# architector1324/micro-raytracer

Measured on AMD Instinct MI355X. Metric: Msamples/sec (res x spp), higher is better.
Workload: dtype f32

## Files before the change

micro_raytracer_amd/csrc/mrt_math.h:

```cpp
#pragma once

#include <stdint.h>

#if defined(__HIPCC__) || defined(__HIP__)
#define MRT_HD __host__ __device__ inline __attribute__((always_inline))
#define MRT_HD_NOINLINE __host__ __device__
#else
#define MRT_HD inline __attribute__((always_inline))
#define MRT_HD_NOINLINE
#endif

namespace mrt {

typedef uint32_t u32;
typedef int32_t i32;

MRT_HD u32 f2u(float f) { return __builtin_bit_cast(u32, f); }
MRT_HD float u2f(u32 u) { return __builtin_bit_cast(float, u); }
MRT_HD float fabs_(float x) { return __builtin_fabsf(x); }
MRT_HD float floor_(float x) { return __builtin_floorf(x); }
MRT_HD float trunc_(float x) { return __builtin_truncf(x); }

#if defined(__HIP_DEVICE_COMPILE__) && !defined(MRT_GENERIC_IEEE)
#define MRT_FAST_IEEE 1
MRT_HD bool wave_all(bool ok) { return __builtin_amdgcn_ballot_w64(!ok) == 0ull; }
#else
MRT_HD bool wave_all(bool ok) { return ok; }
#endif
constexpr float kWinLo = 0x1p-40f, kWinHi = 0x1p+40f;
MRT_HD bool in_window(float x) { const float a = fabs_(x); return a >= kWinLo && a <= kWinHi; }
MRT_HD bool in_window_pos(float x) { return x >= kWinLo && x <= kWinHi; }

#if defined(MRT_FAST_IEEE)
MRT_HD float sqrt_core_(float x)
{
    const float s = __builtin_amdgcn_sqrtf(x);
    const float sd = u2f(f2u(s) - 1u), su = u2f(f2u(s) + 1u);
    const float vd = __builtin_fmaf(-sd, s, x), vu = __builtin_fmaf(-su, s, x);
    float r = (0.0f >= vd) ? sd : s;
    r = (0.0f < vu) ? su : r;
    return r;
}
MRT_HD float rcp_refined_(float d)
{
    const float r0 = __builtin_amdgcn_rcpf(d);
    const float e = __builtin_fmaf(-d, r0, 1.0f);
    return __builtin_fmaf(e, r0, r0);
}
MRT_HD float div_core_(float n, float d, float r)
{
    const float q0 = n * r;
    const float q1 = __builtin_fmaf(__builtin_fmaf(-d, q0, n), r, q0);
    return __builtin_fmaf(__builtin_fmaf(-d, q1, n), r, q1);
}
#endif

MRT_HD float sqrt_(float x)
{
#if defined(MRT_FAST_IEEE)
    if (wave_all(in_window_pos(x))) return sqrt_core_(x);
#endif
    return __builtin_sqrtf(x);
}
MRT_HD float recip_(float x)
{
#if defined(MRT_FAST_IEEE)
    if (wave_all(in_window(x))) return div_core_(1.0f, x, rcp_refined_(x));
#endif
    return 1.0f / x;
}
MRT_HD float div_(float a, float b)
{
#if defined(MRT_FAST_IEEE)
    if (wave_all(in_window(a) && in_window(b))) return div_core_(a, b, rcp_refined_(b));
#endif
    return a / b;
}
MRT_HD void div2_(float a0, float a1, float b, float &q0, float &q1)
{
#if defined(MRT_FAST_IEEE)
    if (wave_all(in_window(a0) && in_window(a1) && in_window(b))) {
        const float r = rcp_refined_(b);
        q0 = div_core_(a0, b, r);
        q1 = div_core_(a1, b, r);
        return;
    }
#endif
    q0 = a0 / b;
    q1 = a1 / b;
}
MRT_HD float recip_sqrt_(float m)
{
#if defined(MRT_FAST_IEEE)
    if (wave_all(in_window_pos(m))) {
        const float s = sqrt_core_(m);
        return div_core_(1.0f, s, rcp_refined_(s));
    }
#endif
    return 1.0f / __builtin_sqrtf(m);
}
MRT_HD float rcp_fast(float x)
{
#if defined(__HIP_DEVICE_COMPILE__)
    return __builtin_amdgcn_rcpf(x);
#else
    return 1.0f / x;
#endif
}
MRT_HD float fma_(float a, float b, float c) { return __builtin_fmaf(a, b, c); }
MRT_HD float fma_fast(float a, float b, float c)
{
#if defined(__HIP_DEVICE_COMPILE__)
    return __builtin_fmaf(a, b, c);
#else
    return a * b + c;
#endif
}

constexpr float kPi = 3.14159274101257324f;
constexpr float kPiO2 = 1.57079637050628662f;
constexpr float kPiO4 = 0.785398185253143311f;
constexpr float kInf = __builtin_huge_valf();

MRT_HD float qnan() { return u2f(0x7fc00000u); }

#if defined(__HIP_DEVICE_COMPILE__)
MRT_HD float fmax_(float a, float b) { return __builtin_fmaxf(a, b); }
MRT_HD float fmin_(float a, float b) { return __builtin_fminf(a, b); }
#else
MRT_HD float fmax_(float a, float b)
{
    if (a != a) return b;
    if (b != b) return a;
    if (a == b) return (f2u(a) & 0x80000000u) ? b : a;
    return a < b ? b : a;
}
MRT_HD float fmin_(float a, float b)
{
    if (a != a) return b;
    if (b != b) return a;
    if (a == b) return (f2u(a) & 0x80000000u) ? a : b;
    return b < a ? b : a;
}
#endif

MRT_HD void sincos_(float x, float &s, float &c)
{
    if (!(fabs_(x) <= 65536.0f)) { s = qnan(); c = qnan(); return; }
    const float kf = floor_(fma_(x, 0.636619746685028076f, 0.5f));
    float r = fma_(-kf, 1.5703125f, x);
    r = fma_(-kf, 4.83751296997070312e-4f, r);
    r = fma_(-kf, 7.54978995489188216e-8f, r);
    const float z = r * r;
    const float sp = fma_(fma_(fma_(-1.9515295891e-4f, z, 8.3321608736e-3f), z, -1.6666654611e-1f) * z, r, r);
    const float cp = fma_(fma_(fma_(2.443315711809948e-5f, z, -1.388731625493765e-3f), z, 4.166664568298827e-2f) * z, z,
                          fma_(-0.5f, z, 1.0f));
    const int q = (int)kf & 3;
    float ss = (q & 1) ? cp : sp;
    float cc = (q & 1) ? sp : cp;
    if (q & 2) ss = -ss;
    if ((q + 1) & 2) cc = -cc;
    s = ss;
    c = cc;
}

MRT_HD float asin_core_(float a)
{
    const float z = a * a;
    const float p = fma_(fma_(fma_(fma_(4.2163199048e-2f, z, 2.4181311049e-2f), z, 4.5470025998e-2f), z, 7.4953002686e-2f), z, 1.6666752422e-1f);
    return fma_(p * z, a, a);
}

MRT_HD float acos_(float x)
{
    const float ax = fabs_(x);
    const bool big = ax > 0.5f;
    const float s = sqrt_(0.5f * (1.0f - ax));
    const float p = asin_core_(big ? s : x);
    const float two_p = 2.0f * p;
    const float r_big = (x > 0.0f) ? two_p : kPi - two_p;
    return big ? r_big : kPiO2 - p;
}

MRT_HD float atan_pos_(float t)
{
    float y0, x;
    if (t > 2.414213562373095f) { y0 = kPiO2; x = -recip_(t); }
    else if (t > 0.4142135623730950f) { y0 = kPiO4; x = div_(t - 1.0f, t + 1.0f); }
    else { y0 = 0.0f; x = t; }
    const float z = x * x;
    const float p = fma_(fma_(fma_(8.05374449538e-2f, z, -1.38776856032e-1f), z, 1.99777106478e-1f), z, -3.33329491539e-1f);
    return y0 + fma_(p * z, x, x);
}

MRT_HD float atan2_(float y, float x)
{
    if (x != x || y != y) return qnan();
    const float ay = fabs_(y), ax = fabs_(x);
    float a;
    if (ax == 0.0f) {
        if (ay == 0.0f) return 0.0f;
        a = kPiO2;
    } else if (ay == kInf && ax == kInf) {
        a = kPiO4;
    } else {
        a = atan_pos_(div_(ay, ax));
    }
    if (x < 0.0f) a = kPi - a;
    return (y < 0.0f) ? -a : a;
}

MRT_HD float pow_(float xf, float yf)
{
    if (yf == 0.0f) return 1.0f;
    if (xf != xf || yf != yf) return qnan();
    if (xf < 0.0f) return qnan();
    if (xf == 0.0f) return (yf > 0.0f) ? 0.0f : kInf;
    if (xf == kInf) return (yf > 0.0f) ? kInf : 0.0f;
    if (xf == 1.0f) return 1.0f;
    if (yf == kInf) return (xf > 1.0f) ? kInf : 0.0f;
    if (yf == -kInf) return (xf > 1.0f) ? 0.0f : kInf;

    const double x = (double)xf;
    const uint64_t bits = __builtin_bit_cast(uint64_t, x);
    int e = (int)((bits >> 52) & 0x7ff) - 1023;
    double m = __builtin_bit_cast(double, (bits & 0x000fffffffffffffULL) | 0x3ff0000000000000ULL);
    if (m > 1.4142135623730951) { m = m * 0.5; e = e + 1; }
    const double r = (m - 1.0) / (m + 1.0);
    const double r2 = r * r;
    double p = 1.0 / 23.0;
    p = p * r2 + 1.0 / 21.0;
    p = p * r2 + 1.0 / 19.0;
    p = p * r2 + 1.0 / 17.0;
    p = p * r2 + 1.0 / 15.0;
    p = p * r2 + 1.0 / 13.0;
    p = p * r2 + 1.0 / 11.0;
    p = p * r2 + 1.0 / 9.0;
    p = p * r2 + 1.0 / 7.0;
    p = p * r2 + 1.0 / 5.0;
    p = p * r2 + 1.0 / 3.0;
    p = p * r2 + 1.0;
    const double lnm = 2.0 * r * p;
    const double log2x = (double)e + lnm * 1.4426950408889634;
    const double t = (double)yf * log2x;
    if (t >= 129.0) return kInf;
    if (t <= -151.0) return 0.0f;
    const double kf = __builtin_floor(t + 0.5);
    const double f = (t - kf) * 0.6931471805599453;
    double q = 1.0 / 6227020800.0;
    q = q * f + 1.0 / 479001600.0;
    q = q * f + 1.0 / 39916800.0;
    q = q * f + 1.0 / 3628800.0;
    q = q * f + 1.0 / 362880.0;
    q = q * f + 1.0 / 40320.0;
    q = q * f + 1.0 / 5040.0;
    q = q * f + 1.0 / 720.0;
    q = q * f + 1.0 / 120.0;
    q = q * f + 1.0 / 24.0;
    q = q * f + 1.0 / 6.0;
    q = q * f + 0.5;
    q = q * f + 1.0;
    q = q * f + 1.0;
    const int k = (int)kf;
    const double scale = __builtin_bit_cast(double, (uint64_t)(k + 1023) << 52);
    return (float)(q * scale);
}

MRT_HD u32 mix32(u32 x)
{
    x ^= x >> 16; x *= 0x7feb352du; x ^= x >> 15; x *= 0x846ca68bu; x ^= x >> 16;
    return x;
}
constexpr u32 kGold = 0x9E3779B9u;
MRT_HD u32 path_key(u32 seed_lo, u32 seed_hi, u32 pixel, u32 sample)
{
    return mix32((mix32(pixel + seed_lo) ^ seed_hi) + sample * kGold);
}
MRT_HD u32 draw_u32(u32 pk, u32 dim) { return mix32(pk + (dim + 1u) * kGold); }
MRT_HD float u32_to_unit(u32 u) { return (float)(u >> 9) * 1.1920928955078125e-7f; }

enum : u32 { DIM_LENS_X = 0, DIM_LENS_Z = 1, DIM_BOUNCE0 = 2, DIMS_PER_BOUNCE = 8 };
enum : u32 { SL_REFL_COIN = 0, SL_REFL_U1, SL_REFL_U2, SL_OPAC_COIN, SL_REFR_COIN, SL_REFR_U1, SL_REFR_U2, SL_EMIT_COIN };

MRT_HD bool bernoulli(float p, u32 u)
{
    if (p == 1.0f) return true;
    return u < (u32)(p * 4294967296.0f);
}

MRT_HD i32 total_key(float t)
{
    if (t != t) return (i32)0x80000000u;
    i32 i = (i32)f2u(t);
    i ^= (i32)(((u32)(i >> 31)) >> 1);
    return i;
}

}
```

micro_raytracer_amd/csrc/mrt_trace.h:

```cpp
#pragma once
#include "mrt_scene.h"

namespace mrt {

#ifndef MRT_LEAF_QUEUE
#define MRT_LEAF_QUEUE 8u
#endif
constexpr u32 kLeafQueue = MRT_LEAF_QUEUE;

#ifndef MRT_PROBE
#define MRT_PROBE(phase)
#endif
#ifndef MRT_COUNT
#define MRT_COUNT(counter)
#endif
#ifndef MRT_PROBE_INST
#define MRT_PROBE_INST(i)
#endif
#if defined(MRT_PHASE_TIMING) && defined(__HIP_DEVICE_COMPILE__)
#define MRT_TICK(slot) do { const unsigned long long now_ = __builtin_amdgcn_s_memtime(); phase_ticks[slot] += now_ - phase_last; phase_last = now_; } while (0)
#define MRT_TICK_DECL unsigned long long phase_ticks[4] = {0ull, 0ull, 0ull, 0ull}; unsigned long long phase_last = __builtin_amdgcn_s_memtime()
#define MRT_TICK_OUT(dst) do { for (int k_ = 0; k_ < 4; ++k_) (dst)[k_] = phase_ticks[k_]; } while (0)
#else
#define MRT_TICK(slot)
// ... 728 lines not shown
                MRT_COUNT(CT_TBVH_TRI_HIT);
                u32 sl, sh;
                if (!memb_candidate<ANY>(S, C, tri0, root, id, ro, m, pos, sl, sh)) continue;
                if (ANY) return true;
                tri_take(best, t, id, sl, sh, t0, i0, t1, i1);
            }
        }
        return best.any;
    }

    count_fallback(P, 7);
    MRT_PROBE_FALLBACK(ro, rd, dd);
    return mesh_isect_ref<ANY, FEAT>(S, mesh, ro, rd, m, pos, t0, i0, t1, i1);
}

#if defined(__HIP_DEVICE_COMPILE__)
MRT_HD u32 wave_uniform(u32 v) { return (u32)__builtin_amdgcn_readfirstlane((int)v); }
#else
MRT_HD u32 wave_uniform(u32 v) { return v; }
#endif
template <bool ANY, u32 FEAT, bool UNIFORM = false>
MRT_HD bool isect_instance(const Scn &S, const RayPre &ray, u32 i, const F4 &ia, const F4 &ib, float &t0, float &t1, i32 &i0, i32 &i1, const float *X0 = nullptr)
{
    const float *F = S.U;
    const Params &P = *S.P;
    const V3 pos = v3(ia.x, ia.y, ia.z);
    const u32 tag = (UNIFORM && (FEAT & F_TRI)) ? wave_uniform(f2u(ib.x)) : f2u(ib.x);
    const u32 kind = (UNIFORM && (FEAT & F_IDENT)) ? wave_uniform(tag & TAG_KIND_MASK) : (tag & TAG_KIND_MASK);
    const bool ident = (FEAT & F_IDENT) ? true : (tag & TAG_IDENT) != 0;
    const float *X = (FEAT & F_IDENT) ? X0 : F + P.off_xf + (tag >> TAG_XF_SHIFT);
    const V3 ro = add(pos, xf_vec(X, ident, sub(ray.o, pos)));
    const bool fast_d = (FEAT & F_IDENT) ? true : (ident && ray.d_ok);
    V3 rd = ray.d, m = ray.m;
    float dd = ray.dd;
    if (!fast_d) {
        rd = xf_full(X, ray.d);
        if constexpr (FEAT & F_BOX) m = recip_patched(rd);
        dd = dot(rd, rd);
    }
    t0 = 0.0f; t1 = 0.0f; i0 = -1; i1 = -1;
    if (kind == KIND_SPHERE) return sphere_isect(ia.w, sub(ro, pos), rd, dd, t0, t1);
    if (kind == KIND_PLANE) { const bool h = plane_isect(v3(ib.y, ib.z, ib.w), ia.w, ro, rd, t0); t1 = t0; return h; }
    if ((FEAT & F_BOX) && kind == KIND_BOX) return box_isect(v3(ia.w, ib.y, ib.z), ro, m, pos, t0, t1);
    if (FEAT & F_TRI) {
        const float *R = F + P.off_rend + ldu(F, P.off_instx + i * INSTX_WORDS + INSTX_REND) * REND_WORDS;
        if (kind == KIND_TRIANGLE) {
            const bool h = tri_isect(add(ld3(R, REND_GEO), pos), ld3(R, REND_GEO + 3), ld3(R, REND_GEO + 6), ro, rd, t0);
            t1 = t0;
            return h;
        }
        if ((FEAT & F_BOX) && kind == KIND_MESH) return mesh_isect<ANY, FEAT>(S, ldu(R, REND_GEO), ro, rd, dd, m, pos, t0, i0, t1, i1);
    }
    return false;
}

#if defined(__HIP_DEVICE_COMPILE__)
#define MRT_ARM_END(name) asm volatile("; axis scan: end of arm " name)
#define MRT_FORGET_SCALAR(v) asm volatile("" : "+s"(v))
#else
#define MRT_ARM_END(name)
#define MRT_FORGET_SCALAR(v)
#endif

template <bool V> struct BoolTag { static constexpr bool value = V; };

template <bool ANY, u32 FEAT>
MRT_HD bool trace(const Scn &S, const RayPre &ray_, Hit &best)
{
    const float *F = S.U;
    const Params &P = *S.P;
    i32 best_key = 0x7fffffff;
    best.rend = -1; best.inst = 0; best.t0 = 0.0f; best.t1 = 0.0f; best.i0 = -1; best.i1 = -1;
    const float *I = F + P.off_inst;

    if (ANY) { MRT_COUNT(CT_TRACE_ANY); } else { MRT_COUNT(CT_TRACE); }
    const float *X0 = nullptr;
    RayPre ray_i = ray_;
    if constexpr (FEAT & F_IDENT) {
        X0 = F + P.off_xf + (ldu(I, INST_TAG) >> TAG_XF_SHIFT);
        if (!ray_.d_ok) {
            ray_i.d = xf_full(X0, ray_.d);
            if constexpr (FEAT & F_BOX) ray_i.m = recip_patched(ray_i.d);
            ray_i.dd = dot(ray_i.d, ray_i.d);
        }
    }
    const RayPre &ray = ray_i;
    auto consider = [&](u32 i, const F4 &ia, const F4 &ib, auto in_order, auto uniform) -> bool {
        float t0, t1;
        MRT_COUNT(CT_LIN_TEST);
        MRT_PROBE_INST(i);
        i32 i0, i1;
        if (!isect_instance<ANY, FEAT, decltype(uniform)::value>(S, ray, i, ia, ib, t0, t1, i0, i1, X0)) return false;
        if (ANY) return true;
        const i32 key = total_key(t0);
        const unsigned long long pair = ((unsigned long long)((u32)key ^ 0x80000000u) << 32) | i;
        const unsigned long long best_pair = ((unsigned long long)((u32)best_key ^ 0x80000000u) << 32) | (best.rend < 0 ? 0xffffffffu : best.inst);
        const bool better = decltype(in_order)::value ? key < best_key : pair < best_pair;
        if (better) {
            best_key = key;
            best.rend = 0; best.inst = i; best.t1 = t1; best.i0 = i0; best.i1 = i1;
            if constexpr ((FEAT & F_BVH) != 0) best.t0 = t0;
        }
        return false;
    };
    using InOrder = BoolTag<(FEAT & F_BVH) == 0>;
    using AnyOrder = BoolTag<false>;
    using Shared = BoolTag<true>;
    using PerLane = BoolTag<false>;

    const bool bvh = (FEAT & F_BVH) != 0;
    const u32 n = bvh ? P.n_lin : P.n_inst;
    bool scanned = false;
    if constexpr (!ANY && FEAT == F_IDENT) {
        const V3 o = ray_.o, d = ray_.d;
        const bool tame = (int)in_window(d.x) & (int)in_window(d.y) & (int)in_window(d.z) & (int)(fabs_(o.x) <= kAxisMax) & (int)(fabs_(o.y) <= kAxisMax) &
                          (int)(fabs_(o.z) <= kAxisMax);
        auto off0 = [](float x) { return (int)(x == 0.0f) | (int)(fabs_(x) >= kWinLo); };
        const bool near0 = !(off0(o.x) & off0(o.y) & off0(o.z));
        bool axis = false;
        if (P.axis_scan && n && wave_all(tame)) {
            MRT_COUNT(CT_AXIS_SCAN);
            axis = wave_all(!near0);
            if (!axis) { MRT_COUNT(CT_AXIS_REDO); }
        }
        if (axis) {
            scanned = true;
            const float *A = F + P.off_axis;
#if defined(MRT_FAST_IEEE)
            const V3 r = v3(rcp_refined_(d.x), rcp_refined_(d.y), rcp_refined_(d.z));
#else
            const V3 r = v3(0.0f, 0.0f, 0.0f);
#endif
            auto plane = [&](u32 i, float ok, float dk, float rk, float pk, float sd) {
                const float ro = pk + (ok - pk);
                const float num = -(ro + sd);
#if defined(MRT_FAST_IEEE)
                const float tt = div_core_(num, dk, rk);
#else
                const float tt = num / dk;
#endif
                (void)rk;
                const i32 kb = (i32)f2u(tt);
                if (kb > 0 && kb < best_key) { best_key = kb; best.inst = i; best.t1 = tt; }
            };
            const float a = ray_.dd, den = 2.0f * a;
            const bool a_mid = (int)(a > 0.0f) & (int)(a < 1e18f);
#if defined(MRT_FAST_IEEE)
            const bool den_ok = in_window(den);
            const float rden = rcp_refined_(den);
#endif
            auto sphere = [&](u32 i, const F4 &ia) {
                const V3 pos = v3(ia.x, ia.y, ia.z);
                const V3 ro = add(pos, sub(o, pos));
                const V3 oo = sub(ro, pos);
                const float b = 2.0f * dot(oo, d);
                const float c = dot(oo, oo) - ia.w;
                const float disc = b * b - 4.0f * a * c;
                if (disc < 0.0f) return;
                if (b > 1e-20f && a_mid && disc >= 0.0f) return;
                MRT_PROBE(PH_SPHERE_MATH);
#if defined(MRT_FAST_IEEE)
                const float sqc = sqrt_core_(disc);
                const float m0 = -b - sqc, m1 = -b + sqc;
                const float least = __builtin_fminf(__builtin_fminf(disc, fabs_(m0)), fabs_(m1));
                const float most = __builtin_fmaxf(__builtin_fmaxf(disc, fabs_(m0)), fabs_(m1));
                if (wave_all((int)(least >= kWinLo) & (int)(most <= kWinHi) & (int)den_ok)) {
                    const float q0 = div_core_(m0, den, rden), q1 = div_core_(m1, den, rden);
                    const i32 kb = (i32)f2u(q0);
                    if (kb > 0 && kb < best_key) { best_key = kb; best.inst = i; best.t1 = q1; }
                    return;
                }
#endif
                const float sq = __builtin_sqrtf(disc);
                const float q0 = (-b - sq) / den, q1 = (-b + sq) / den;
                if (q0 < 0.0f) return;
                const i32 key = total_key(q0);
                if (key < best_key) { best_key = key; best.inst = i; best.t1 = q1; }
            };
            auto test = [&](u32 i, const F4 &ia, const F2 &ax) {
                MRT_COUNT(CT_LIN_TEST);
                MRT_PROBE_INST(i);
                u32 code = wave_uniform(f2u(ax.x));
                if (code == 1u) { plane(i, o.x, d.x, r.x, ia.x, ax.y); MRT_ARM_END("x"); }
                MRT_FORGET_SCALAR(code);
                if (code == 2u) { plane(i, o.y, d.y, r.y, ia.y, ax.y); MRT_ARM_END("y"); }
                MRT_FORGET_SCALAR(code);
                if (code == 3u) { plane(i, o.z, d.z, r.z, ia.z, ax.y); MRT_ARM_END("z"); }
                MRT_FORGET_SCALAR(code);
                if (code == 0u) { sphere(i, ia); MRT_ARM_END("sphere"); }
            };
            u32 j = 0;
            F4 a0 = ld4(I, 0), b0;
            F2 c0 = ld2(A, 0), e0;
            for (;;) {
                b0 = ld4(I, (j + 1u) * INST_WORDS); e0 = ld2(A, (j + 1u) * AXIS_WORDS);
                test(j, a0, c0);
                if (++j >= n) break;
                a0 = ld4(I, (j + 1u) * INST_WORDS); c0 = ld2(A, (j + 1u) * AXIS_WORDS);
                test(j, b0, e0);
                if (++j >= n) break;
            }
            best.rend = best_key != 0x7fffffff ? 0 : -1;
        }
    }
    if (scanned) {
    } else if (!bvh && !(FEAT & F_TRI) && n) {
        u32 j = 0;
        F4 a0 = ld4(I, 0), a1 = ld4(I, 4), b0 = a0, b1 = a1;
        for (;;) {
            if (j + 1u < n) { b0 = ld4(I, (j + 1u) * INST_WORDS); b1 = ld4(I, (j + 1u) * INST_WORDS + 4); }
            if (consider(j, a0, a1, InOrder(), Shared())) return true;
            if (++j >= n) break;
            if (j + 1u < n) { a0 = ld4(I, (j + 1u) * INST_WORDS); a1 = ld4(I, (j + 1u) * INST_WORDS + 4); }
            if (consider(j, b0, b1, InOrder(), Shared())) return true;
            if (++j >= n) break;
        }
    } else if (n) {
        const float *Lst = F + P.off_lin;
        u32 cur = bvh ? ldu(Lst, 0) : 0u;
        F4 qa = ld4(I, cur * INST_WORDS), qb = ld4(I, cur * INST_WORDS + 4);
        for (u32 j = 0; j < n; ++j) {
            const F4 ia = qa, ib = qb;
            const u32 i = cur;
            if (j + 1 < n) {
                cur = bvh ? ldu(Lst, j + 1) : j + 1;
                qa = ld4(I, cur * INST_WORDS); qb = ld4(I, cur * INST_WORDS + 4);
            }
            if (consider(i, ia, ib, InOrder(), Shared())) return true;
        }
    }

    if constexpr (bvh) {
        const bool cull = cull_ok(ray_.o, ray_.dd);
        CullRay R = cull_ray(ray_.d);
        const float *N0 = F + P.off_bvh;
        u32 node = P.n_bvh_nodes ? 0u : BVH_END;
        float mg;
        {
            const F4 ra = ld4(N0, 0), rb = ld4(N0, 4);
            const V3 r = sub(v3(ra.x, ra.y, ra.z), ray_.o);
            const float ext = fmax_(fmax_(fabs_(r.x) + ra.w, fabs_(r.y) + rb.x), fabs_(r.z) + rb.y);
            const float obig = fmax_(fmax_(fabs_(ray_.o.x), fabs_(ray_.o.y)), fabs_(ray_.o.z));
            const float ksq = fmin_(P.inst_ksq * ext, 4e-3f) * MRT_MARGIN_SCALE;
            mg = fma_fast(P.inst_k * MRT_MARGIN_SCALE + ksq, ext, fma_fast(P.inst_kpos * MRT_MARGIN_SCALE, obig + obig + ext, 1e-6f * MRT_MARGIN_SCALE));
        }
        cull_from(R, ray_.o, mg);
        for (;;) {
            u32 leaf_a = 0u, leaf_b = 0u;
            bool walking = node != BVH_END;
            const float far = (!ANY && best.rend >= 0 && best.t0 >= 0.0f) ? best.t0 + 1e-3f * best.t0 + mg : kInf;
            while (walking) {
                const F4 na = ld4(N0, node * BVH_WORDS), nb = ld4(N0, node * BVH_WORDS + 4);
                MRT_COUNT(CT_BVH_NODE);
                const u32 skip = f2u(nb.z), leaf = f2u(nb.w);
                float tn;
                bool hit_node = cull_hit(R, na.x, na.y, na.z, na.w, nb.x, nb.y, tn);
                if (!ANY) hit_node = hit_node && !(tn > far);
                hit_node = hit_node || !cull;
                const u32 cand = hit_node ? leaf : 0u;
                const bool have_a = leaf_a != 0u;
                leaf_b |= have_a ? cand : 0u;
                leaf_a |= have_a ? 0u : cand;
                node = (hit_node && leaf == 0u) ? node + 1u : skip;
                walking = node != BVH_END && leaf_b == 0u;
            }
            if (leaf_a == 0u) break;
            const u32 cnt_a = leaf_a >> 24, first_a = leaf_a & 0xffffffu, cnt_b = leaf_b >> 24, first_b = leaf_b & 0xffffffu;
            for (u32 k = 0; k < cnt_a + cnt_b; ++k) {
                const u32 i = ldu(F, P.off_bvhinst + (k < cnt_a ? first_a + k : first_b + (k - cnt_a)));
                if (consider(i, ld4(I, i * INST_WORDS), ld4(I, i * INST_WORDS + 4), AnyOrder(), PerLane())) return true;
            }
        }
    }
    if (best.rend < 0) return false;
    if constexpr ((FEAT & F_BVH) == 0) {
        const i32 k = best_key;
        best.t0 = u2f((u32)(k ^ (i32)(((u32)(k >> 31)) >> 1)));
    }
    best.rend = (i32)ldu(S.F, P.off_instx + best.inst * INSTX_WORDS + INSTX_REND);
    return true;
}

struct Obj {
    const float *R, *IX, *X;
    V3 pos;
    bool ident;
    u32 kind;
};
MRT_HD Obj obj_of(const Scn &S, const Hit &h)
{
    Obj o;
    const float *I = S.F + S.P->off_inst + h.inst * INST_WORDS;
    const u32 tag = ldu(I, INST_TAG);
    o.R = S.F + S.P->off_rend + (u32)h.rend * REND_WORDS;
    o.IX = S.F + S.P->off_instx + h.inst * INSTX_WORDS;
    o.X = S.F + S.P->off_xf + (tag >> TAG_XF_SHIFT);
    o.pos = ld3(I, INST_POS);
    o.ident = (tag & TAG_IDENT) != 0;
    o.kind = tag & TAG_KIND_MASK;
    return o;
}
MRT_HD V3 to_object(const Obj &o, V3 hp) { return add(o.pos, xf_vec(o.X, o.ident, sub(hp, o.pos))); }

struct Bary { float b1, b2; bool ok; };
MRT_HD bool finite_(float x) { return (f2u(x) & 0x7f800000u) != 0x7f800000u; }
MRT_HD Bary tri_bary(V3 p, V3 v0, V3 e1, V3 e2)
{
    const V3 q = sub(p, v0);
    const float d00 = dot(e1, e1), d01 = dot(e1, e2), d11 = dot(e2, e2), d20 = dot(q, e1), d21 = dot(q, e2);
    const float den = d00 * d11 - d01 * d01;
    Bary b;
    b.b1 = div_(d11 * d20 - d01 * d21, den);
    b.b2 = div_(d00 * d21 - d01 * d20, den);
    b.ok = den != 0.0f && finite_(den) && finite_(b.b1) && finite_(b.b2);
    return b;
}
MRT_HD float bary_mix(const Bary &b, float a0, float a1, float a2) { return a0 + (b.b1 * (a1 - a0) + b.b2 * (a2 - a0)); }
MRT_HD V3 vattr_normal(V3 p, V3 v0, V3 e1, V3 e2, const float *vn)
{
    const Bary b = tri_bary(p, v0, e1, e2);
    const V3 n = v3(bary_mix(b, vn[0], vn[3], vn[6]), bary_mix(b, vn[1], vn[4], vn[7]), bary_mix(b, vn[2], vn[5], vn[8]));
    const bool good = b.ok && finite_(n.x) && finite_(n.y) && finite_(n.z) && !(n.x == 0.0f && n.y == 0.0f && n.z == 0.0f);
    return good ? n : cross(e1, e2);
}
MRT_HD UV vattr_uv(V3 p, V3 v0, V3 e1, V3 e2, const float *uv)
{
    const Bary b = tri_bary(p, v0, e1, e2);
    UV r;
    r.x = fract_(b.ok ? bary_mix(b, uv[0], uv[2], uv[4]) : uv[0]);
    if (r.x < 0.0f) r.x = 1.0f + r.x;
    r.y = fract_(b.ok ? bary_mix(b, uv[1], uv[3], uv[5]) : uv[1]);
    if (r.y < 0.0f) r.y = 1.0f + r.y;
    return r;
}
template <u32 FEAT>
MRT_HD const float *vattr_tri(const Scn &S, const Obj &o, i32 tri_idx)
{
    if (o.kind == KIND_TRIANGLE) return o.R + REND_GEO;
    const float *M = S.F + S.P->off_mesh + ldu(o.R, REND_GEO) * MESH_WORDS;
    return ((FEAT & F_DEEP) ? S.G : S.F) + S.P->off_tri + (ldu(M, MESH_TRI0) + (u32)tri_idx) * TRI_WORDS;
}
template <u32 N4>
MRT_HD void vattr_row(const Scn &S, const Obj &o, i32 tri_idx, u32 first4, float *out)
{
    const float *A = S.G + ldu(o.R, REND_VATTR) + (o.kind == KIND_TRIANGLE ? 0u : (u32)tri_idx) * VATTR_WORDS + first4 * 4u;
    for (u32 k = 0; k < N4; ++k) { const F4 v = ld4(A, k * 4u); out[k * 4u] = v.x; out[k * 4u + 1u] = v.y; out[k * 4u + 2u] = v.z; out[k * 4u + 3u] = v.w; }
}

template <u32 FEAT>
MRT_HD V3 hit_normal(const Scn &S, const Obj &o, V3 n_hit, i32 tri_idx)
{
    if (o.kind == KIND_PLANE) return ld3(o.IX, INSTX_PLANE_NW);
    if constexpr (FEAT & F_VATTR) {
        if ((o.kind == KIND_TRIANGLE || o.kind == KIND_MESH) && (ldu(o.R, REND_FLAGS) & RF_HAS_VN)) {
            const float *T = vattr_tri<FEAT>(S, o, tri_idx);
            float a[12];
            vattr_row<3>(S, o, tri_idx, 0u, a);
            return norm(xf_vec(o.X, o.ident, vattr_normal(sub(n_hit, o.pos), ld3(T, 0), ld3(T, 3), ld3(T, 6), a + VATTR_VN)));
        }
    }
    V3 n = v3(0.0f, 0.0f, 0.0f);
    if (o.kind == KIND_SPHERE) n = sub(n_hit, o.pos);
    else if ((FEAT & F_BOX) && o.kind == KIND_BOX) n = box_normal(ld3(o.R, REND_GEO + 3), n_hit, o.pos);
    else if ((FEAT & F_TRI) && o.kind == KIND_TRIANGLE) n = cross(ld3(o.R, REND_GEO + 3), ld3(o.R, REND_GEO + 6));
    else if (FEAT & F_TRI) {
        const float *M = S.F + S.P->off_mesh + ldu(o.R, REND_GEO) * MESH_WORDS;
        const float *T = ((FEAT & F_DEEP) ? S.G : S.F) + S.P->off_tri + (ldu(M, MESH_TRI0) + (u32)tri_idx) * TRI_WORDS;
        n = cross(ld3(T, 3), ld3(T, 6));
    }
    return norm(xf_vec(o.X, o.ident, n));
}

template <u32 FEAT>
MRT_HD UV hit_uv(const Scn &S, const Obj &o, V3 n_hit, i32 tri_idx)
{
    UV r;
    if (o.kind == KIND_SPHERE) {
        const V3 v = norm(sub(n_hit, o.pos));
        r.x = 0.5f + div_(0.5f * atan2_(v.x, -v.y), kPi);
        r.y = 0.5f - 0.5f * v.z;
    } else if (o.kind == KIND_PLANE) {
        r.x = fract_(n_hit.x + 0.5f);
        if (r.x < 0.0f) r.x = 1.0f + r.x;
        r.y = fract_(n_hit.y + 0.5f);
        if (r.y < 0.0f) r.y = 1.0f + r.y;
    } else if (o.kind == KIND_BOX) {
        r = box_uv(ld3(o.R, REND_GEO + 3), n_hit, o.pos);
    } else {
        r.x = 0.0f; r.y = 0.0f;
        if constexpr (FEAT & F_VATTR) {
            if (ldu(o.R, REND_FLAGS) & RF_HAS_UV) {
                const float *T = vattr_tri<FEAT>(S, o, tri_idx);
                float a[8];
                vattr_row<2>(S, o, tri_idx, 2u, a);
                r = vattr_uv(sub(n_hit, o.pos), ld3(T, 0), ld3(T, 3), ld3(T, 6), a + (VATTR_UV - 8u));
            }
        }
    }
    return r;
}

struct Surf {
    const float *M;
    bool maps;
    UV uv;
};
template <u32 FEAT>
MRT_HD Surf surf_of(const Scn &S, const Hit &h, const Obj &o, V3 n_hit, i32 tri_idx)
{
    Surf s;
    s.M = S.F + S.P->off_mat + (u32)h.rend * MAT_WORDS;
    s.maps = false;
    s.uv.x = 0.0f; s.uv.y = 0.0f;
    if constexpr (FEAT & F_MAPS) {
        s.maps = (ldu(o.R, REND_FLAGS) & RF_HAS_MAPS) != 0;
        if (s.maps) s.uv = hit_uv<FEAT>(S, o, n_hit, tri_idx);
    }
    return s;
}
template <u32 FEAT>
MRT_HD float surf_scalar(const Scn &S, const Surf &s, u32 slot, u32 field)
{
    if (s.maps) {
        const i32 id = (i32)ldu(s.M, MAT_MAP + slot);
        if (id >= 0) {
            if constexpr (FEAT & F_ENV) { const u32 fl = ldu(s.M, MAT_FLAGS); if (fl & MATF_BILINEAR) return tex_fetch_bilinear<FEAT>(S, id, s.uv, fl).x; }
            return tex_fetch<FEAT>(S, id, s.uv).x;
        }
    }
    return s.M[field];
}
template <u32 FEAT>
MRT_HD V3 surf_color(const Scn &S, const Surf &s)
{
    const V3 albedo = ld3(s.M, MAT_ALBEDO);
    if (s.maps) {
        const i32 id = (i32)ldu(s.M, MAT_MAP + MAP_TEX);
        if (id >= 0) {
            if constexpr (FEAT & F_ENV) { const u32 fl = ldu(s.M, MAT_FLAGS); if (fl & MATF_BILINEAR) return hadam(albedo, tex_fetch_bilinear<FEAT>(S, id, s.uv, fl)); }
            return hadam(albedo, tex_fetch<FEAT>(S, id, s.uv));
        }
    }
    return albedo;
}

MRT_HD V3 rand_normal(V3 n, float r, float u1, float u2)
{
    const float phi = u2 * 2.0f * kPi;
    const float cth = 1.0f - 2.0f * u1;
    const float sth = sqrt_((4.0f * u1) * (1.0f - u1));
    float sphi, cphi;
    sincos_(phi, sphi, cphi);
    const V3 v = v3(sth * cphi, sth * sphi, cth);
    return norm(add(n, muls(v, r)));
}

MRT_HD bool refract(V3 d, float eta, V3 n, V3 &out)
{
    const float cosv = dot(neg(n), d);
    const float k = 1.0f - (eta * eta) * (1.0f - cosv * cosv);
    if (k < 0.0f) return false;
    out = add(muls(d, eta), muls(n, cosv * eta + sqrt_(k)));
    return true;
}

MRT_HD V3 pixel_focus(const Params &P, float cx, float cy)
{
    const float uvx = div_(P.aspect * (cx - 0.5f * P.w), P.w);
    const float uvy = div_(cy - 0.5f * P.h, P.h);
    const V3 dir = norm(v3(uvx, P.inv2tan, -uvy));
    const V3 cam = v3(P.cam_pos[0], P.cam_pos[1], P.cam_pos[2]);
    const V3 orig = add(cam, muls(dir, kE));
    return add(orig, muls(dir, P.foc));
}

MRT_HD V3 lens_pos(const Params &P, u32 pk)
{
    const float u1 = u32_to_unit(draw_u32(pk, DIM_LENS_X));
    const float u2 = u32_to_unit(draw_u32(pk, DIM_LENS_Z));
    return v3(P.cam_pos[0] + (u1 - 0.5f) * P.aprt, P.cam_pos[1], P.cam_pos[2] + (u2 - 0.5f) * P.aprt);
}

MRT_HD void camera_ray(const Params &P, const float *camF, V3 focus, u32 pk, V3 &o, V3 &d)
{
    const float u1 = u32_to_unit(draw_u32(pk, DIM_LENS_X));
    const float u2 = u32_to_unit(draw_u32(pk, DIM_LENS_Z));
    const V3 pos = v3(P.cam_pos[0] + (u1 - 0.5f) * P.aprt, P.cam_pos[1], P.cam_pos[2] + (u2 - 0.5f) * P.aprt);
    const V3 new_dir = norm(sub(focus, pos));
    if (P.cam_ident && nzfin3(new_dir)) d = new_dir;
    else d = m3mul(camF + 9, m3mul(camF, new_dir));
    o = add(pos, muls(d, kE));
}

MRT_HD void camera_ray_centre(const Params &P, const float *camF, V3 focus, V3 &o, V3 &d)
{
    const V3 pos = v3(P.cam_pos[0], P.cam_pos[1], P.cam_pos[2]);
    const V3 new_dir = norm(sub(focus, pos));
    if (P.cam_ident && nzfin3(new_dir)) d = new_dir;
    else d = m3mul(camF + 9, m3mul(camF, new_dir));
    o = add(pos, muls(d, kE));
}

constexpr u32 kThr080 = 3435973836u;

MRT_HD u32 dim_of(u32 bounce, u32 slot) { return DIM_BOUNCE0 + bounce * DIMS_PER_BOUNCE + slot; }

MRT_HD bool coin(float p, u32 pk, u32 dim)
{
    if (p == 1.0f) return true;
    if (!(p > 0.0f)) return false;
    return draw_u32(pk, dim) < (u32)(p * 4294967296.0f);
}

enum : u32 { ST_FOCUS = 0, ST_PIXKEY = 3, ST_CHUNK = 4, ST_SEND = 5, ST_WORD = 6, ST_SLOTS = 7, ST_P0Y = 7, ST_P0Z = 8, ST_PK = 9, ST_SLOTS_HIT = 10, ST_T = 10, ST_L = 13, ST_SLOTS_TL = 16 };
constexpr bool tl_in_stash(u32 feat, u32 ) { return (feat & F_COLD) && (feat & F_BVH) && !(feat & F_TRI); }
constexpr bool hit_in_stash(u32 feat, u32 threads) { return tl_in_stash(feat, threads); }
constexpr u32 stash_slots_for(u32 feat, u32 threads) { return tl_in_stash(feat, threads) ? (u32)ST_SLOTS_TL : (u32)ST_SLOTS; }
struct RegStash {
    static constexpr bool in_lds = false;
    static constexpr u32 threads = 0;
    float v[ST_SLOTS_TL];
    MRT_HD void put(u32 slot, float x) { v[slot] = x; }
    MRT_HD float get(u32 slot) const { return v[slot]; }
};
#if defined(__HIPCC__) || defined(__HIP__)
template <u32 THREADS>
struct LdsStash {
    static constexpr bool in_lds = true;
    static constexpr u32 threads = THREADS;
    lds_vfloat *base;
    MRT_HD void put(u32 slot, float x) { base[slot * THREADS] = x; }
    MRT_HD float get(u32 slot) const { return base[slot * THREADS]; }
};
#endif
template <class St> MRT_HD void st_put3(St &st, u32 slot, V3 v) { st.put(slot, v.x); st.put(slot + 1, v.y); st.put(slot + 2, v.z); }
template <class St> MRT_HD V3 st_get3(const St &st, u32 slot) { return v3(st.get(slot), st.get(slot + 1), st.get(slot + 2)); }


struct LaneJob {
    u32 k;
    u32 word;
};

struct CameraRays { static constexpr bool supplied = false; };
struct SuppliedRay {
    static constexpr bool supplied = true;
    V3 o, d;
    u32 key;
};

template <u32 FEAT, class Stash, class Prim = CameraRays>
MRT_HD void render_pixel(const Scn &S, Stash &st, u32 x, u32 y, const LaneJob &job, u32 &segments, unsigned long long *ticks = nullptr,
                         const Prim &prim = Prim())
{
    MRT_TICK_DECL;
    const Params &P = *S.P;
    u32 pixel;
    if constexpr (Prim::supplied) pixel = prim.key; else pixel = y * P.nw + x;
    const u32 pix_key = mix32(pixel + P.seed_lo) ^ P.seed_hi;
    const V3 sky_init = v3(P.sky_init[0], P.sky_init[1], P.sky_init[2]);
    const u32 s_base = P.sample_base, s_stop = P.sample_base + P.n_samples;
    const u32 g0 = s_base / kChunk;
    const u32 n_chunks = (s_stop - 1u) / kChunk - g0 + 1u;
    const bool planes1 = P.to_planes != 0u;
    const bool direct = P.k_split == 1u && !planes1;
    if constexpr (!Prim::supplied) st_put3(st, ST_FOCUS, pixel_focus(P, (float)x, (float)y));

    st.put(ST_PIXKEY, u2f(pix_key));
    st.put(ST_WORD, u2f(job.word));
    st.put(ST_CHUNK, u2f(job.k));
    u32 s = (g0 + job.k) * kChunk;
    {
        u32 e = s_stop - s > kChunk ? s + kChunk : s_stop;
        if (s < s_base || planes1) s = s_base;
        if (planes1) e = s_base + 1u;
        st.put(ST_SEND, u2f(e));
    }
    bool alive = planes1 ? job.k == 0u : job.k < n_chunks;
    V3 csum = v3(0.0f, 0.0f, 0.0f);
    u32 pk = 0, b = 0;
    V3 o = v3(0, 0, 0), d = v3(0, 1, 0);
    constexpr bool kTL = Stash::in_lds && tl_in_stash(FEAT, Stash::threads);
    constexpr bool kHit = Stash::in_lds && hit_in_stash(FEAT, Stash::threads);
    V3 T_ = v3(1, 1, 1), L_ = v3(0, 0, 0);
    auto getT = [&]() { if constexpr (kTL) return st_get3(st, ST_T); else return T_; };
    auto getL = [&]() { if constexpr (kTL) return st_get3(st, ST_L); else return L_; };
    auto setT = [&](V3 v) { if constexpr (kTL) st_put3(st, ST_T, v); else T_ = v; };
    auto setL = [&](V3 v) { if constexpr (kTL) st_put3(st, ST_L, v); else L_ = v; };
    setT(v3(1, 1, 1)); setL(v3(0, 0, 0));
    float pwr = 1.0f;
    u32 seg = 0;
    if (alive) {
        pk = mix32(pix_key + s * kGold);
        if constexpr (kHit) st.put(ST_PK, u2f(pk));
        if constexpr (Prim::supplied) { o = prim.o; d = prim.d; }
        else camera_ray(P, S.F + P.off_cam, st_get3(st, ST_FOCUS), pk, o, d);
    }

    while (alive) {
        MRT_PROBE(PH_ITER);
        const RayPre ray = ray_pre<FEAT>(o, d);
        Hit h;
        ++seg;
        V3 contrib = v3(0.0f, 0.0f, 0.0f);
        bool ended = false;
        V3 X = v3(0.0f, 1.0f, 0.0f);
        V3 base = o;
        MRT_TICK(3);
        const bool hit_any = trace<false, FEAT>(S, ray, h);
        MRT_TICK(0);
        if (!hit_any) {
            bool env = false;
            if constexpr (FEAT & F_ENV) {
                if (P.off_env != 0u) {
                    float sky_pwr;
                    const V3 e = env_color<FEAT>(S, d, sky_pwr);
                    contrib = (b == 0) ? e : add(getL(), hadam(getT(), muls(e, sky_pwr)));
                    env = true;
                }
            }
            if (!env) contrib = (b == 0) ? v3(P.sky[0], P.sky[1], P.sky[2]) : add(getL(), hadam(getT(), sky_init));
            ended = true;
        } else {
            MRT_PROBE(PH_SHADE);
            const Obj ob = obj_of(S, h);
            if constexpr (kHit) pk = f2u(st.get(ST_PK));
            const V3 p0_ = add(o, muls(d, h.t0));
            if constexpr (kHit) { st.put(ST_P0Y, p0_.y); st.put(ST_P0Z, p0_.z); }
            auto p0 = [&]() { if constexpr (kHit) return v3(p0_.x, st.get(ST_P0Y), st.get(ST_P0Z)); else return p0_; };
            const V3 nh0 = to_object(ob, p0_);
            const Surf sf0 = surf_of<FEAT>(S, h, ob, nh0, h.i0);
            const float opacity0 = surf_scalar<FEAT>(S, sf0, MAP_OPACITY, MAT_OPACITY);
            const float metal_c = sf0.M[MAT_METAL];

            bool refr = coin(fmin_(1.0f - opacity0, 0.85f), pk, dim_of(b, SL_OPAC_COIN));
            V3 hp, hn;
            Surf sfh;
            u32 pass = 0;
            for (;;) {
                if (pass == 0) { MRT_PROBE(PH_SCATTER1); } else { MRT_PROBE(PH_SCATTER2); }
                ++pass;
                if (refr) { MRT_PROBE(PH_REFRACT); }
                if (ob.kind != KIND_PLANE) { MRT_PROBE(PH_NORMAL_NONPLANE); }
                hp = refr ? add(o, muls(d, h.t1)) : p0();
                const V3 nhh = refr ? to_object(ob, hp) : nh0;
                hn = hit_normal<FEAT>(S, ob, nhh, refr ? h.i1 : h.i0);
                sfh = sf0;
                if (refr) sfh = surf_of<FEAT>(S, h, ob, nhh, h.i1);
                float rough = surf_scalar<FEAT>(S, sfh, MAP_ROUGH, MAT_ROUGH);
                const float opac = refr ? surf_scalar<FEAT>(S, sfh, MAP_OPACITY, MAT_OPACITY) : opacity0;
                const u32 dbase = dim_of(b, refr ? SL_REFR_COIN : SL_REFL_COIN);
                if (metal_c == 0.0f && opac != 0.0f && draw_u32(pk, dbase) < kThr080) rough = 1.0f;
                const V3 nn = rand_normal(hn, rough, u32_to_unit(draw_u32(pk, dbase + 1u)), u32_to_unit(draw_u32(pk, dbase + 2u)));
                if (refr) {
                    const float eta = 1.0f + 0.5f * surf_scalar<FEAT>(S, sfh, MAP_GLASS, MAT_GLASS);
                    if (refract(d, eta, nn, X)) break;
                    refr = false;
                    continue;
                }
                X = reflect(d, nn);
                break;
            }
            base = hp;

            const V3 color = surf_color<FEAT>(S, sfh);
            const float emit = surf_scalar<FEAT>(S, sfh, MAP_EMIT, MAT_EMIT);
            if (coin(emit, pk, dim_of(b, SL_EMIT_COIN))) {
                MRT_PROBE(PH_EMIT_END);
                contrib = add(getL(), hadam(getT(), color));
                ended = true;
            } else {
                if ((FEAT & F_LIGHTS) && P.n_light) {
                    V3 l_col = v3(0.0f, 0.0f, 0.0f);
                    const float rough_h = surf_scalar<FEAT>(S, sfh, MAP_ROUGH, MAT_ROUGH);
                    const float metal_h = surf_scalar<FEAT>(S, sfh, MAP_METAL, MAT_METAL);
                    for (u32 li = 0; li < P.n_light; ++li) {
                        const float *Lt = S.F + P.off_light + li * LIGHT_WORDS;
                        const bool point = ldu(Lt, LIGHT_KIND) == LK_POINT;
                        const V3 lv = ld3(Lt, LIGHT_V);
                        const V3 ln = point ? norm(sub(lv, hp)) : lv;
                        const float diff = fmax_(dot(ln, hn), 0.0f);
                        const float sp = fmax_(dot(d, reflect(ln, hn)), 0.0f);
                        const float s2 = sp * sp, s4 = s2 * s2, s8 = s4 * s4, s16 = s8 * s8, s32 = s16 * s16;
                        const float spec = s32 * (1.0f - rough_h);
                        const V3 o_col = muls(color, 1.0f - metal_h);
                        V3 t = hadam(muls(o_col, diff), ld3(Lt, LIGHT_COLOR));
                        t = v3(t.x + spec, t.y + spec, t.z + spec);
                        const V3 term = muls(t, Lt[LIGHT_PWR]);
                        if (term.x == 0.0f && term.y == 0.0f && term.z == 0.0f) continue;
                        const V3 ph0 = p0();
                        const V3 ls = point ? norm(sub(lv, ph0)) : lv;
                        const V3 so = add(ph0, muls(ls, kE));
                        Hit hs;
                        MRT_TICK(1);
                        const bool blocked = trace<true, FEAT>(S, ray_pre<FEAT>(so, ls), hs);
                        MRT_TICK(2);
                        if (blocked) continue;
                        l_col = add(l_col, term);
                    }
                    setL(add(getL(), hadam(getT(), muls(l_col, pwr))));
                }
                setT(hadam(getT(), muls(v3(0.5f + color.x, 0.5f + color.y, 0.5f + color.z), pwr)));
                pwr = pwr * P.q;
                ++b;
                if (b > P.bounce) {
                    contrib = add(getL(), hadam(getT(), sky_init));
                    ended = true;
                }
            }
        }
    
        MRT_TICK(1);
        bool from_camera = false;
        if (ended) {
            csum = add(csum, contrib);
            ++s;
            if (s == f2u(st.get(ST_SEND))) {
                u32 j = f2u(st.get(ST_CHUNK));
                if (direct) {
                    float *q = P.accum + f2u(st.get(ST_WORD));
                    q[0] += csum.x; q[1] += csum.y; q[2] += csum.z;
                } else {
                    float *q = P.partial + ((size_t)j * P.partial_stride + f2u(st.get(ST_WORD)));
                    q[0] = csum.x; q[1] = csum.y; q[2] = csum.z;
                }
                csum = v3(0.0f, 0.0f, 0.0f);
                u32 e;
                if (planes1) {
                    j += 1u;
                    alive = s < s_stop;
                    e = s + 1u;
                } else {
                    j += P.k_split;
                    alive = j < n_chunks;
                    s = (g0 + j) * kChunk;
                    e = s_stop - s > kChunk ? s + kChunk : s_stop;
                }
                st.put(ST_CHUNK, u2f(j));
                st.put(ST_SEND, u2f(e));
            }
            if (alive) {
                MRT_PROBE(PH_REGEN);
                pk = mix32(f2u(st.get(ST_PIXKEY)) + s * kGold);
                if constexpr (kHit) st.put(ST_PK, u2f(pk));
                if constexpr (!Prim::supplied) {
                    base = lens_pos(P, pk);
                    X = sub(st_get3(st, ST_FOCUS), base);
                }
                setT(v3(1.0f, 1.0f, 1.0f)); setL(v3(0.0f, 0.0f, 0.0f));
                pwr = 1.0f; b = 0;
                from_camera = true;
            }
        }
        V3 nd = norm(X);
        if (from_camera && !(P.cam_ident && nzfin3(nd))) nd = m3mul(S.F + P.off_cam + 9, m3mul(S.F + P.off_cam, nd));
        o = add(base, muls(nd, kE));
        d = nd;
        if constexpr (Prim::supplied) { if (from_camera) { o = prim.o; d = prim.d; } }
    }
    segments = seg;
    (void)ticks;
    MRT_TICK_OUT(ticks);
}

}
```

Measured before the change: 10500.

## Add specialized path-tracing loop for scenes without lights, maps or env

Adds a compile-time specialized render loop for feature sets limited to box/triangle/BVH/identity, which skips light, texture and environment handling. Camera regeneration and scatter share one random-draw and ray-finalization path to reduce divergence. For identity-transform scenes the object transform is skipped via a templated Obj/xf path, and the refraction exit point is computed only when some lane in the wave refracts. This adds code size and a second loop that must match the general loop's semantics.

```diff
diff --git a/micro_raytracer_amd/csrc/mrt_math.h b/micro_raytracer_amd/csrc/mrt_math.h
--- a/micro_raytracer_amd/csrc/mrt_math.h
+++ b/micro_raytracer_amd/csrc/mrt_math.h
@@ -24,8 +24,10 @@
 #if defined(__HIP_DEVICE_COMPILE__) && !defined(MRT_GENERIC_IEEE)
 #define MRT_FAST_IEEE 1
 MRT_HD bool wave_all(bool ok) { return __builtin_amdgcn_ballot_w64(!ok) == 0ull; }
+MRT_HD bool wave_any(bool some) { return __builtin_amdgcn_ballot_w64(some) != 0ull; }
 #else
 MRT_HD bool wave_all(bool ok) { return ok; }
+MRT_HD bool wave_any(bool some) { return some; }
 #endif
 constexpr float kWinLo = 0x1p-40f, kWinHi = 0x1p+40f;
 MRT_HD bool in_window(float x) { const float a = fabs_(x); return a >= kWinLo && a <= kWinHi; }
diff --git a/micro_raytracer_amd/csrc/mrt_trace.h b/micro_raytracer_amd/csrc/mrt_trace.h
--- a/micro_raytracer_amd/csrc/mrt_trace.h
+++ b/micro_raytracer_amd/csrc/mrt_trace.h
@@ -1054,6 +1054,31 @@
 }
 MRT_HD V3 to_object(const Obj &o, V3 hp) { return add(o.pos, xf_vec(o.X, o.ident, sub(hp, o.pos))); }
 
+MRT_HD const float *ident_xf0(const Scn &S) { return S.F + S.P->off_xf + (ldu(S.F + S.P->off_inst, INST_TAG) >> TAG_XF_SHIFT); }
+template <bool IDENT>
+MRT_HD Obj obj_of_t(const Scn &S, const Hit &h)
+{
+    if constexpr (!IDENT) return obj_of(S, h);
+    Obj o;
+    const float *I = S.F + S.P->off_inst + h.inst * INST_WORDS;
+    o.R = S.F + S.P->off_rend + (u32)h.rend * REND_WORDS;
+    o.IX = S.F + S.P->off_instx + h.inst * INSTX_WORDS;
+    o.X = nullptr;
+    o.pos = ld3(I, INST_POS);
+    o.ident = true;
+    o.kind = ldu(I, INST_TAG) & TAG_KIND_MASK;
+    return o;
+}
+template <bool IDENT>
+MRT_HD V3 xf_obj(const Scn &S, const Obj &o, V3 v)
+{
+    if constexpr (!IDENT) return xf_vec(o.X, o.ident, v);
+    if (nzfin3_product(v)) return v;
+    return xf_full(ident_xf0(S), v);
+}
+template <bool IDENT>
+MRT_HD V3 to_object_t(const Scn &S, const Obj &o, V3 hp) { return add(o.pos, xf_obj<IDENT>(S, o, sub(hp, o.pos))); }
+
 struct Bary { float b1, b2; bool ok; };
 MRT_HD bool finite_(float x) { return (f2u(x) & 0x7f800000u) != 0x7f800000u; }
 MRT_HD Bary tri_bary(V3 p, V3 v0, V3 e1, V3 e2)
@@ -1099,7 +1124,7 @@
     for (u32 k = 0; k < N4; ++k) { const F4 v = ld4(A, k * 4u); out[k * 4u] = v.x; out[k * 4u + 1u] = v.y; out[k * 4u + 2u] = v.z; out[k * 4u + 3u] = v.w; }
 }
 
-template <u32 FEAT>
+template <u32 FEAT, bool IDENT = false>
 MRT_HD V3 hit_normal(const Scn &S, const Obj &o, V3 n_hit, i32 tri_idx)
 {
     if (o.kind == KIND_PLANE) return ld3(o.IX, INSTX_PLANE_NW);
@@ -1108,7 +1133,7 @@
             const float *T = vattr_tri<FEAT>(S, o, tri_idx);
             float a[12];
             vattr_row<3>(S, o, tri_idx, 0u, a);
-            return norm(xf_vec(o.X, o.ident, vattr_normal(sub(n_hit, o.pos), ld3(T, 0), ld3(T, 3), ld3(T, 6), a + VATTR_VN)));
+            return norm(xf_obj<IDENT>(S, o, vattr_normal(sub(n_hit, o.pos), ld3(T, 0), ld3(T, 3), ld3(T, 6), a + VATTR_VN)));
         }
     }
     V3 n = v3(0.0f, 0.0f, 0.0f);
@@ -1120,7 +1145,7 @@
         const float *T = ((FEAT & F_DEEP) ? S.G : S.F) + S.P->off_tri + (ldu(M, MESH_TRI0) + (u32)tri_idx) * TRI_WORDS;
         n = cross(ld3(T, 3), ld3(T, 6));
     }
-    return norm(xf_vec(o.X, o.ident, n));
+    return norm(xf_obj<IDENT>(S, o, n));
 }
 
 template <u32 FEAT>
@@ -1226,11 +1251,13 @@
     return add(orig, muls(dir, P.foc));
 }
 
+MRT_HD V3 lens_at(const Params &P, float u1, float u2)
+{
+    return v3(P.cam_pos[0] + (u1 - 0.5f) * P.aprt, P.cam_pos[1], P.cam_pos[2] + (u2 - 0.5f) * P.aprt);
+}
 MRT_HD V3 lens_pos(const Params &P, u32 pk)
 {
-    const float u1 = u32_to_unit(draw_u32(pk, DIM_LENS_X));
-    const float u2 = u32_to_unit(draw_u32(pk, DIM_LENS_Z));
-    return v3(P.cam_pos[0] + (u1 - 0.5f) * P.aprt, P.cam_pos[1], P.cam_pos[2] + (u2 - 0.5f) * P.aprt);
+    return lens_at(P, u32_to_unit(draw_u32(pk, DIM_LENS_X)), u32_to_unit(draw_u32(pk, DIM_LENS_Z)));
 }
 
 MRT_HD void camera_ray(const Params &P, const float *camF, V3 focus, u32 pk, V3 &o, V3 &d)
@@ -1295,6 +1322,7 @@
 };
 
 struct CameraRays { static constexpr bool supplied = false; };
+constexpr bool end_before_scatter(u32 feat) { return (feat & ~(u32)(F_BOX | F_TRI | F_BVH | F_IDENT)) == 0u; }
 struct SuppliedRay {
     static constexpr bool supplied = true;
     V3 o, d;
@@ -1349,6 +1377,134 @@
         else camera_ray(P, S.F + P.off_cam, st_get3(st, ST_FOCUS), pk, o, d);
     }
 
+    if constexpr (end_before_scatter(FEAT)) {
+    static_assert(!kTL && !kHit, "the 6-wave stash kernels carry lights and maps");
+    constexpr bool kId = (FEAT & F_IDENT) != 0;
+    float q_pwr = P.q;
+    u32 bounce_max = P.bounce;
+    u32 k_split = P.k_split;
+    MRT_FORGET_SCALAR(q_pwr); MRT_FORGET_SCALAR(bounce_max); MRT_FORGET_SCALAR(k_split);
+    while (alive) {
+        MRT_PROBE(PH_ITER);
+        const RayPre ray = ray_pre<FEAT>(o, d);
+        Hit h;
+        ++seg;
+        V3 contrib = v3(0.0f, 0.0f, 0.0f);
+        bool ended = false;
+        MRT_TICK(3);
+        const bool hit_any = trace<false, FEAT>(S, ray, h);
+        MRT_TICK(0);
+        const float *M = S.F + P.off_mat;
+        bool refr = false;
+        if (!hit_any) {
+            contrib = (b == 0) ? v3(P.sky[0], P.sky[1], P.sky[2]) : add(L_, hadam(T_, sky_init));
+            ended = true;
+        } else {
+            MRT_PROBE(PH_SHADE);
+            M += (u32)h.rend * MAT_WORDS;
+            refr = coin(fmin_(1.0f - M[MAT_OPACITY], 0.85f), pk, dim_of(b, SL_OPAC_COIN));
+            const V3 color = ld3(M, MAT_ALBEDO);
+            if (coin(M[MAT_EMIT], pk, dim_of(b, SL_EMIT_COIN))) {
+                MRT_PROBE(PH_EMIT_END);
+                contrib = add(L_, hadam(T_, color));
+                ended = true;
+            } else {
+                T_ = hadam(T_, muls(v3(0.5f + color.x, 0.5f + color.y, 0.5f + color.z), pwr));
+                pwr = pwr * q_pwr;
+                ++b;
+                if (b > bounce_max) {
+                    contrib = add(L_, hadam(T_, sky_init));
+                    ended = true;
+                }
+            }
+        }
+
+        MRT_TICK(1);
+        bool from_camera = false;
+        if (ended) {
+            csum = add(csum, contrib);
+            ++s;
+            if (s == f2u(st.get(ST_SEND))) {
+                u32 j = f2u(st.get(ST_CHUNK));
+                if (direct) {
+                    float *q = P.accum + f2u(st.get(ST_WORD));
+                    q[0] += csum.x; q[1] += csum.y; q[2] += csum.z;
+                } else {
+                    float *q = P.partial + ((size_t)j * P.partial_stride + f2u(st.get(ST_WORD)));
+                    q[0] = csum.x; q[1] = csum.y; q[2] = csum.z;
+                }
+                csum = v3(0.0f, 0.0f, 0.0f);
+                u32 e;
+                if (planes1) {
+                    j += 1u;
+                    alive = s < s_stop;
+                    e = s + 1u;
+                } else {
+                    j += k_split;
+                    alive = j < n_chunks;
+                    s = (g0 + j) * kChunk;
+                    e = s_stop - s > kChunk ? s + kChunk : s_stop;
+                }
+                st.put(ST_CHUNK, u2f(j));
+                st.put(ST_SEND, u2f(e));
+            }
+            if (alive) {
+                MRT_PROBE(PH_REGEN);
+                pk = mix32(f2u(st.get(ST_PIXKEY)) + s * kGold);
+                T_ = v3(1.0f, 1.0f, 1.0f); L_ = v3(0.0f, 0.0f, 0.0f);
+                pwr = 1.0f; b = 0;
+                from_camera = true;
+            }
+        }
+        MRT_TICK(3);
+        u32 dbase = dim_of(b - 1u, refr ? SL_REFR_COIN : SL_REFL_COIN);
+        const u32 ddim = from_camera ? (u32)DIM_LENS_X : dbase + 1u;
+        float u1 = u32_to_unit(draw_u32(pk, ddim)), u2 = u32_to_unit(draw_u32(pk, ddim + 1u));
+        V3 X = v3(0.0f, 1.0f, 0.0f);
+        V3 base = o;
+        if (from_camera) {
+            if constexpr (!Prim::supplied) {
+                base = lens_at(P, u1, u2);
+                X = sub(st_get3(st, ST_FOCUS), base);
+            }
+        } else if (!ended) {
+            const Obj ob = obj_of_t<kId>(S, h);
+            const V3 p0 = add(o, muls(d, h.t0));
+            const V3 nh0 = to_object_t<kId>(S, ob, p0);
+            const float metal_c = M[MAT_METAL], opac = M[MAT_OPACITY];
+            V3 hp = p0, nhh = nh0;
+            i32 ti = h.i0;
+            if (wave_any(refr)) {
+                const V3 p1 = add(o, muls(d, h.t1));
+                const V3 nh1 = to_object_t<kId>(S, ob, p1);
+                if (refr) { hp = p1; nhh = nh1; ti = h.i1; }
+            }
+            for (u32 pass = 0;; ++pass) {
+                if (pass == 0) { MRT_PROBE(PH_SCATTER1); } else { MRT_PROBE(PH_SCATTER2); }
+                if (refr) { MRT_PROBE(PH_REFRACT); }
+                if (ob.kind != KIND_PLANE) { MRT_PROBE(PH_NORMAL_NONPLANE); }
+                const V3 hn = hit_normal<FEAT, kId>(S, ob, nhh, ti);
+                float rough = M[MAT_ROUGH];
+                if (metal_c == 0.0f && opac != 0.0f && draw_u32(pk, dbase) < kThr080) rough = 1.0f;
+                const V3 nn = rand_normal(hn, rough, u1, u2);
+                if (!refr) { X = reflect(d, nn); break; }
+                const float eta = 1.0f + 0.5f * M[MAT_GLASS];
+                if (refract(d, eta, nn, X)) break;
+                refr = false;
+                hp = p0; nhh = nh0; ti = h.i0;
+                dbase = dim_of(b - 1u, SL_REFL_COIN);
+                u1 = u32_to_unit(draw_u32(pk, dbase + 1u)); u2 = u32_to_unit(draw_u32(pk, dbase + 2u));
+            }
+            base = hp;
+        }
+        MRT_TICK(1);
+        V3 nd = norm(X);
+        if (from_camera && !(P.cam_ident && nzfin3(nd))) nd = m3mul(S.F + P.off_cam + 9, m3mul(S.F + P.off_cam, nd));
+        o = add(base, muls(nd, kE));
+        d = nd;
+        if constexpr (Prim::supplied) { if (from_camera) { o = prim.o; d = prim.d; } }
+    }
+    } else
     while (alive) {
         MRT_PROBE(PH_ITER);
         const RayPre ray = ray_pre<FEAT>(o, d);
```

Result: faster. 11120 (median of 6 runs) (+6.0%).
